# bldeng/AA-ADMM

Measured on AMD Instinct MI355X. Metric: ADMM iters/sec + time-to-eps (primal+dual residual), higher is better.
Workload: dtype f64

## Files before the change

aa-admm_amd/csrc/elastic.cpp:

```cpp
#include "elastic.hpp"

#include <algorithm>
#include <chrono>
#include <cmath>
#include <cstdio>
#include <cstdlib>
#include <cstring>
#include <memory>
#include <numeric>
#include <set>

#include "dense_gpu.hpp"
#include "spd_direct.hpp"

namespace aa {

ElasticSolver::~ElasticSolver() {
    if (fr_ev0_) { (void)hipEventDestroy(fr_ev0_); (void)hipEventDestroy(fr_ev1_); }
    if (fr_ev2_) (void)hipEventDestroy(fr_ev2_);
    drop_graph();
    if (ev_fork_) (void)hipEventDestroy(ev_fork_);
    if (ev_join_) (void)hipEventDestroy(ev_join_);
    if (side_) (void)hipStreamDestroy(side_);
    for (auto& kv : kstats_)
// ... 621 lines not shown
        auto pf = make_part_factor(P > 1 ? comm_ : nullptr, rank_, s());
        F = factor_on_device(A, tree, s(), pf.get());
    } catch (const Error&) {
        throw;
    } catch (const std::runtime_error& e) {
        throw Error(ERR_NUMERIC, e.what());
    }
    pipe_z_ = st_.variant == AA_VARIANT_Z && st_.acceleration_type == 1;
    if (const char* e = std::getenv("AA_Z_PIPELINE")) pipe_z_ = pipe_z_ && e[0] != '0';
    conc_ = pipe_z_ && !comm_;
    if (const char* e = std::getenv("AA_CONCURRENT")) conc_ = conc_ && e[0] != '0';
    win_u_ = conc_;
    if (const char* e = std::getenv("AA_Z_WINDOW")) win_u_ = win_u_ && e[0] != '0';
    comb_fused_ = true;
    if (const char* e = std::getenv("AA_COMB_FUSED")) comb_fused_ = e[0] != '0';
    stamp("factor");
    solver_.default_branches = (P == 1 && st_.variant == AA_VARIANT_Z) ? 2 : 1;
    solver_.build(F, s(), P > 1 ? &tree.part : nullptr, rank_, top_beg_, comm_, pipe_z_ ? 2 : 1,
                  st_.variant == AA_VARIANT_Z && st_.acceleration_type == 1);
    stamp("solver build + upload");

    std::vector<HostGroup> owned;
    nbg_ = 0;
    long long zmax = 0;
    if (P > 1) {
        std::vector<int> qpart(n, -1);
        for (int r = 0; r < P; ++r) for (int q = tree.part_beg[r]; q < tree.part_end[r]; ++q) qpart[q] = r;
        std::vector<long long> zr(P, 0);
        std::vector<int> br(P, 0);
        long long rr = 0;
// ... 98 lines not shown
            groups_[gi].d.spos = groups_[gi].spos.p;
        }
        Yslots_ = pos;
    }
    std::vector<double> xs(3 * (size_t)n), ms(n);
    for (int q = 0; q < n; ++q) {
        for (int j = 0; j < 3; ++j) xs[3 * (size_t)q + j] = x_[3 * (size_t)int2node_[q] + j];
        ms[q] = m3_[3 * (size_t)int2node_[q]];
    }
    xs_.upload(xs, s());
    vs_.alloc(3 * (size_t)n); vs_.zero(s());
    mass_.upload(ms, s());
    xfull_.alloc(3 * (size_t)n); xlast_.alloc(3 * (size_t)n); cxfull_.alloc(3 * (size_t)n);
    xfull_.zero(s()); xlast_.zero(s()); cxfull_.zero(s());
    xbar_.alloc(3 * (size_t)nf_); Mxbar_.alloc(3 * (size_t)nf_); b_.alloc(3 * (size_t)nf_);
    if (pipe_z_) b2_.alloc(3 * (size_t)nf_); dx_.alloc(3 * (size_t)nf_);
    z_.alloc(Z_); if (!win_u_) u_.alloc(Z_); y_.alloc(3 * std::max<long long>(1, Yslots_)); du_.alloc(Z_);
    if (st_.variant == AA_VARIANT_Z) { dz_.alloc(Z_); lastz_.alloc(Z_); cz_.alloc(Z_); }
    if (conc_) {
        du2_.alloc(Z_); dz2_.alloc(Z_); dx2_.alloc(3 * (size_t)nf_);
        ctrl_c_.alloc(1);
        lzq2_.alloc(2);
        AA_HIP(hipMemset(lzq2_.p, 0, 2 * sizeof(int)));
        if (!side_) AA_HIP(hipStreamCreateWithFlags(&side_, hipStreamNonBlocking));
        if (!ev_fork_) AA_HIP(hipEventCreateWithFlags(&ev_fork_, hipEventDisableTiming));
        if (!ev_join_) AA_HIP(hipEventCreateWithFlags(&ev_join_, hipEventDisableTiming));
    }
    nbg_ = std::max(1, nbg_);
    red_ab_.alloc(2 * (size_t)nbg_); red_ab_.zero(s());
    if (conc_) { red_c_.alloc(2 * (size_t)nbg_); red_c_.zero(s()); }
    pa_ = red_ab_.p; pb_ = red_ab_.p + nbg_;
    if (comm_) { red_gab_.alloc(2 * (size_t)nbg_); red_gab_.zero(s()); ga_ = red_gab_.p; gb_ = red_gab_.p + nbg_; }
    else { ga_ = pa_; gb_ = pb_; }
    ctrl_.alloc(1);
    lzq_.alloc(2);
    AA_HIP(hipMemset(lzq_.p, 0, 2 * sizeof(int)));
    if (const char* q = std::getenv("AA_LOCAL_QUEUE")) use_queue_ = q[0] != '0';
    lq_ = make_local_queue(ctx_->device, lzq_.p);
    if (conc_) {
        lq2_ = make_local_queue(ctx_->device, lzq2_.p);
    }
    if (const char* q = std::getenv("AA_LQ_STATS"); q && q[0] == '1') {
        lq_stats_.alloc(kLqStats);
        lq_stats_.zero(s());
        lq_.stats = lq_stats_.p;
    }
    if (conc_) lq2_.stats = lq_.stats;
    hist_cap_ = std::max(1, st_.admm_iters);
    hist_prim_.alloc(hist_cap_); hist_comb_.alloc(hist_cap_); hist_rej_.alloc(hist_cap_);
// ... 97 lines not shown
    zero(own_end_, top_beg_);
    if (rank_ != 0) zero(top_beg_, n_);
    comm_->allreduce_sum(v.p, v.p, 3 * (size_t)n_, s());
}

void ElasticSolver::upload_pins() {
    if (!pins_dirty_) return;
    std::vector<double> p(3 * (size_t)np_);
    int q = 0;
    for (auto& kv : pins_) { for (int j = 0; j < 3; ++j) p[3 * q + j] = kv.second[j]; ++q; }
    if (np_) {
        const size_t off = 3 * (size_t)nf_;
        AA_HIP(hipMemcpyAsync(xfull_.p + off, p.data(), p.size() * 8, hipMemcpyHostToDevice, s()));
        AA_HIP(hipMemcpyAsync(xlast_.p + off, p.data(), p.size() * 8, hipMemcpyHostToDevice, s()));
        AA_HIP(hipMemcpyAsync(cxfull_.p + off, p.data(), p.size() * 8, hipMemcpyHostToDevice, s()));
        AA_HIP(hipStreamSynchronize(s()));
    }
    pins_dirty_ = false;
}

void ElasticSolver::ev_begin(const char* name) {
    if (!instrument_) return;
    hipEvent_t e;
    AA_HIP(hipEventCreate(&e));
    AA_HIP(hipEventRecord(e, s()));
    kstats_[name].ev.push_back(e);
}
void ElasticSolver::ev_end(const char* name) { ev_begin(name); }

void ElasticSolver::local_z_all(const double* xfull, const double* u, double* z, double* y, int mode, bool red) {
// ... 100 lines not shown
        launch_aa_reduce(G, aa_cur_.p, Z_, aa_dF_.p, aa_dG_.p, c, aa_red_.p, aa_blocks_, cp, m, s(), ga_, gb_, nbg_,
                         hist_prim_.p, hist_comb_.p, hist_rej_.p);
        reduce_aa();
        launch_aa_solve(c, aag_, aa_blocks_, m, s());
        launch_aa_mix(G, aa_cur_.p, Z_, aa_dF_.p, aa_dG_.p, c, G, m, s(), comb_fused_);
        ev_end("aa");
    } else {
        launch_control(CTL_COMB_UX, c, ga_, gb_, nbg_, accel, hist_prim_.p, hist_comb_.p, hist_rej_.p, s());
    }
}

void ElasticSolver::enqueue_iteration_z(bool accel, int it) {
    const long long nx = 3LL * nf_;
    Ctrl* c = ctrl_.p;
    const bool pipe = accel && pipe_z_;
    double *duc = du_at(it), *dzc = dz_at(it), *dxc = dx_at(it);
    double *dup = du_at(it - 1), *dzp = dz_at(it - 1), *dxp = dx_at(it - 1);
    const bool side = pipe && it > 0 && conc_;
    auto side_pass = [&](hipStream_t st) {
        comb_finish_z(CTL_COMB_ZP, st, ctrl_c_.p, red_c_.p, red_c_.p + nbg_, &lq2_, dup, dzp);
    };
    double* u = u_at(it);
    const double* ui = win_u_ ? dup : u_.p;
    ev_begin("grad");
    for (auto& g : groups_) launch_u_and_y(g.d, xfull_.p, z_.p, u, u, y_.p, nf_, accel ? 1 : 0, 0, c, s(), g.var);
    ev_end("grad");
    ev_begin("rhs");
    launch_rhs(nf_, dt_ptr_.p, nullptr, nullptr, y_.p, Mxbar_.p, pdt2_, b_.p, c, 0, s());
    ev_end("rhs");
    if (pipe && it > 0) {
        ev_begin("solve");
        solver_.solve2(b_.p, xfull_.p, b2_.p, cxfull_.p, c, 0, s());
        ev_end("solve");
        if (side) {
            launch_ctrl_fork(c, ctrl_c_.p, s());
        } else {
            ev_begin("comb");
            comb_finish_z(CTL_COMB_ZP, s(), c, pa_, pb_, &lq_, dup, dzp);
            launch_copy(xfull_.p, dxp, nx, c, 2, s());
            ev_end("comb");
        }
    } else {
        ev_begin(pipe ? "solve1" : "solve");
        solver_.solve(b_.p, xfull_.p, c, 0, s());
        ev_end(pipe ? "solve1" : "solve");
    }
    auto prim_all = [&](const double* xf, const double* z, const double* zref, int redo) {
        int off = 0;
        for (auto& g : groups_) {
            launch_prim_z(g.d, xf, z, zref, nf_, redo, c, pa_, zref ? pb_ : nullptr, off, s());
            off += blocks_for(g.d.count);
        }
    };
    ev_begin("prim");
    prim_all(xfull_.p, z_.p, nullptr, 0);
    ev_end("prim");
    reduce_partials();
    launch_check_restore_z(c, ga_, nbg_, accel, win_u_ ? nullptr : u_.p, xfull_.p, z_.p, dup, dxp, dzp, Z_, nx, s());
    if (accel) {
        ev_begin("reject");
        for (auto& g : groups_) launch_u_and_y(g.d, xfull_.p, z_.p, ui, u, y_.p, nf_, 0, 1, c, s(), g.var);
        launch_rhs(nf_, dt_ptr_.p, nullptr, nullptr, y_.p, Mxbar_.p, pdt2_, b_.p, c, 1, s());
        solver_.solve(b_.p, xfull_.p, c, 1, s());
        prim_all(xfull_.p, z_.p, nullptr, 1);
        reduce_partials();
        ev_end("reject");
    }
    launch_control(CTL_PRIM_FINAL_Z, c, ga_, nullptr, nbg_, accel, hist_prim_.p, hist_comb_.p, hist_rej_.p, s());
    if (accel) {
        const int m = st_.anderson_m;
        auto copy_defaults = [&]() {
            ev_begin("copy");
            launch_copy(dxc, xfull_.p, nx, c, 0, s());
            if (!win_u_) launch_copy(duc, u_.p, Z_, c, 0, s());
            ev_end("copy");
        };
        if (instrument_) copy_defaults();
        ev_begin("local_z");
        local_z_all(xfull_.p, u, dzc, y_.p, LZ_NORMAL, false);
        ev_end("local_z");
        if (side && instrument_) {
            ev_begin("comb");
            side_pass(s());
// ... 40 lines not shown
    ev_end("local_z");
    prim_all(xfull_.p, z_.p, lastz_.p, 0);
    reduce_partials();
    launch_control(CTL_COMB_Z, c, ga_, gb_, nbg_, accel, hist_prim_.p, hist_comb_.p, hist_rej_.p, s());
}

void ElasticSolver::comb_finish_z(int op, hipStream_t st, Ctrl* c, double* pa, double* pb, const LocalQueue* q,
                                  const double* du, const double* dz) {
    const LocalQueue* lq = use_queue_ ? q : nullptr;
    auto fused = [&](const DevGroup& g) { return comb_fused_ && local_z_res_ok(g.d, lq); };
    for (auto& g : groups_) {
        if (fused(g)) launch_local_z_res(g.d, cxfull_.p, du, dz, cz_.p, nf_, c, st, lq, g.var);
        else launch_local_z(g.d, cxfull_.p, du, cz_.p, nullptr, nf_, st_.variant, LZ_NORMAL, c, nullptr, 0, st, lq, g.var,
                            mesh_table(g.d));
    }
    int off = 0;
    for (auto& g : groups_) {
        if (fused(g)) launch_prim_sum(g.d, cz_.p, c, pa, pb, off, st);
        else launch_prim_z(g.d, cxfull_.p, cz_.p, dz, nf_, 0, c, pa, pb, off, st);
        off += blocks_for(g.d.count);
    }
    if (st == s()) {
        reduce_partials();
        launch_control(op, c, ga_, gb_, nbg_, 1, hist_prim_.p, hist_comb_.p, hist_rej_.p, st);
    } else {
        launch_control(op, c, pa, pb, nbg_, 1, hist_prim_.p, hist_comb_.p, hist_rej_.p, st);
    }
}

void ElasticSolver::join_side() {
    if (join_wait_) AA_HIP(hipStreamWaitEvent(s(), ev_join_, 0));
    launch_ctrl_join(ctrl_.p, ctrl_c_.p, xfull_.p, join_dx_, 3LL * nf_, s());
}

void ElasticSolver::enqueue_comb_tail_z(int iters) {
    ev_begin("comb");
// ... 420 lines not shown
```

aa-admm_amd/csrc/elastic.hpp:

```cpp
#pragma once
#include <array>
#include <map>
#include <memory>
#include <string>
#include <vector>

#include "../../include/aa_admm.h"
#include "bending.hpp"
#include "comm.hpp"
#include "common.hpp"
#include "contact_friction.hpp"
#include "direct_solve.hpp"
#include "elastic_kernels.hpp"
#include "mesh_obstacle.hpp"
#include "mesh_refit.hpp"

namespace aa {

struct Context {
    int device = 0;
    hipStream_t stream = nullptr;
};

struct MeshObsBuffers {
// ... 200 lines not shown
    bool join_wait_ = false;
    double* join_dx_ = nullptr;
    void join_side();
    hipStream_t side_ = nullptr;
    hipEvent_t ev_fork_ = nullptr, ev_join_ = nullptr;
    DevBuf<Ctrl> ctrl_c_;
    DevBuf<int> lzq2_;
    LocalQueue lq2_;
    DevBuf<double> red_c_, du2_, dz2_, dx2_;
    double* du_at(int it) { return conc_ && (it & 1) ? du2_.p : du_.p; }
    double* dz_at(int it) { return conc_ && (it & 1) ? dz2_.p : dz_.p; }
    double* dx_at(int it) { return conc_ && (it & 1) ? dx2_.p : dx_.p; }
    bool win_u_ = false;
    double* u_at(int it) { return win_u_ ? du_at(it) : u_.p; }
    bool comb_fused_ = true;

    bool instrument_ = false;
    struct KStat { std::vector<hipEvent_t> ev; double bytes = 0; double total_ms = 0; int launches = 0; };
    std::map<std::string, KStat> kstats_;
    void ev_begin(const char* name);
    void ev_end(const char* name);

    void upload_pins();
    void prologue();
    void enqueue_iteration_ux(bool accel);
    void enqueue_iteration_z(bool accel, int it);
    void comb_finish_z(int op, hipStream_t st, Ctrl* c, double* pa, double* pb, const LocalQueue* q,
                       const double* du, const double* dz);
    void enqueue_comb_tail_z(int iters);
    void enqueue_iterations(int iters, bool accel);
// ... 8 lines not shown
```

aa-admm_amd/csrc/elastic_kernels.hip:

```cpp
#include <algorithm>
#include <cstdlib>

#include "common.hpp"
#include "device_lbfgs.hpp"
#include "device_prox.hpp"
#include "elastic_kernels.hpp"

namespace aa {

namespace {

__device__ __forceinline__ double wave_sum(double v) {
#pragma unroll
    for (int o = 32; o > 0; o >>= 1) v += __shfl_down(v, o, 64);
    return v;
}

__device__ __forceinline__ double block_sum(double v, double* sm) {
    v = wave_sum(v);
    const int lane = threadIdx.x & 63, wid = threadIdx.x >> 6;
    if (lane == 0) sm[wid] = v;
    __syncthreads();
    double r = 0;
    if (threadIdx.x == 0)
// ... 30 lines not shown
__device__ __forceinline__ bool record_iter(Ctrl* c, double* hp, double* hc, int* hr, double comb) {
    const int k = c->nrec;
    if (k < c->cap) {
        hp[k] = c->prim; hc[k] = comb; hr[k] = c->reject;
        if (c->hist_clock) c->hist_clock[k] = (long long)wall_clock64();
    }
    c->nrec = k + 1;
    if (k == 0) c->eps_abs = c->eps_rel * comb;
    return c->eps_rel > 0 && comb <= c->eps_abs;
}

__device__ __forceinline__ bool gated(const Ctrl* c, int gate_reject) {
    if (!c) return false;
    if (c->done) return true;
    return gate_reject && !c->reject;
}

template <int S>
__device__ __forceinline__ void gather_F(const GroupDev& g, int e, const double* __restrict__ xfull, int nf, double* F,
                                         double* Cp) {
    constexpr int NV = shape_nv(S), NC = shape_nc(S);
#pragma unroll
    for (int i = 0; i < 3 * NC; ++i) { F[i] = 0; Cp[i] = 0; }
#pragma unroll
    for (int a = 0; a < NV; ++a) {
        const int v = g.idx[(size_t)a * g.count + e];
        const double x0 = xfull[3 * (size_t)v], x1 = xfull[3 * (size_t)v + 1], x2 = xfull[3 * (size_t)v + 2];
        const bool pin = v >= nf;
#pragma unroll
        for (int c = 0; c < NC; ++c) {
// ... 92 lines not shown
}

template <class... V>
constexpr bool kVar = sizeof...(V) != 0;
__device__ __forceinline__ const GroupVar& var_of(const GroupVar& v) { return v; }
struct ResArgs {
    const double* zref;
};
template <class... V>
constexpr bool kRes = false;
template <class... V>
constexpr bool kRes<ResArgs, V...> = true;
__device__ __forceinline__ const GroupVar& var_of(const ResArgs&, const GroupVar& v) { return v; }
__device__ __forceinline__ const ResArgs& res_of(const ResArgs& r) { return r; }
__device__ __forceinline__ const ResArgs& res_of(const ResArgs& r, const GroupVar&) { return r; }
template <bool VAR>
struct LaneMat {};
template <>
struct LaneMat<true> {
    double mu = 0, lambda = 0, k = 0;
};

template <int S, int HYPER, class... V>
__global__ __launch_bounds__(kBlock) void k_local_z(GroupDev g, const double* __restrict__ xfull,
                                                    const double* __restrict__ u, double* __restrict__ z,
                                                    double* __restrict__ y, int nf, int variant, int mode, Ctrl* ctrl,
                                                    double* red, int red_off, V... gvp) {
    constexpr bool VAR = kVar<V...>;
    if (mode != LZ_INIT && gated(ctrl, mode == LZ_REDO)) return;
    __shared__ double sm[kBlock / 64];
// ... 493 lines not shown
            pa += r * r;
            pb += d * d;
            u[o] += r;
        }
    }
    const double sa = block_sum(pa, sm);
    const double sb = block_sum(pb, sm);
    if (threadIdx.x == 0) { red_a[red_off + blockIdx.x] = sa; red_b[red_off + blockIdx.x] = sb; }
}

template <int S, int HYPER, class... V>
__global__ __launch_bounds__(kBlock) void k_u_and_y(GroupDev g, const double* __restrict__ xfull,
                                                    const double* __restrict__ z, const double* uin, double* u,
                                                    double* __restrict__ y, int nf, int mode, int redo, Ctrl* ctrl,
                                                    V... gvp) {
    constexpr bool VAR = kVar<V...>;
    if (gated(ctrl, redo)) return;
    constexpr int NV = S == kShapeHinge ? 0 : shape_nv(S), D = 3 * shape_nc(S);
    const int e = blockIdx.x * blockDim.x + threadIdx.x;
    if (e >= g.count) return;
    double F[D], Cp[D], zz[D], uu[D];
    const double w = g.w[e];
    const double vol = (NV == 4 && mode == 1) ? g.vol[e] : 0.0;
    double mu = g.mu, lambda = g.lambda, k = g.k;
    if constexpr (VAR && NV == 4) {
        const GroupVar& gv = var_of(gvp...);
        if (mode == 1) { mu = gv.mu[e]; lambda = gv.lambda[e]; k = gv.k[e]; }
    }
#pragma unroll
    for (int i = 0; i < D; ++i) zz[i] = z[g.zoff + (size_t)i * g.count + e];
    if (mode != 1) {
#pragma unroll
        for (int i = 0; i < D; ++i) uu[i] = uin[g.zoff + (size_t)i * g.count + e];
    }
    if (mode == 1) {
        double gr[D];
        if constexpr (NV == 3 || NV == 1 || S == kShapeHinge) {
            if (ctrl) ctrl->fail = 2;
#pragma unroll
            for (int i = 0; i < D; ++i) gr[i] = 0;
        } else if constexpr (HYPER == 0) {
            dev::tet_linear_grad(zz, k * vol, gr);
        } else {
            dev::hyper_psi_grad(g.mat, mu, lambda, zz, gr);
#pragma unroll
            for (int i = 0; i < D; ++i) gr[i] *= vol;
        }
#pragma unroll
        for (int i = 0; i < D; ++i) uu[i] = gr[i] / w;
    }
    if (mode == 0) {
        gather_F<S>(g, e, xfull, nf, F, Cp);
#pragma unroll
        for (int i = 0; i < D; ++i) uu[i] += w * F[i] - w * zz[i];
    } else {
        gather_Cp<S>(g, e, xfull, nf, Cp);
    }
    if (mode != 2) {
#pragma unroll
        for (int i = 0; i < D; ++i) u[g.zoff + (size_t)i * g.count + e] = uu[i];
    }
    write_slots<S>(g, e, nf, w, zz, Cp, uu, y);
}

template <int S>
__global__ __launch_bounds__(kBlock) void k_prim_z(GroupDev g, const double* __restrict__ xfull,
                                                   const double* __restrict__ z, const double* __restrict__ zref,
                                                   int nf, int redo, Ctrl* ctrl, double* red_a, double* red_b,
                                                   int red_off) {
    if (gated(ctrl, redo)) return;
    __shared__ double sm[kBlock / 64];
    constexpr int D = 3 * shape_nc(S);
    const int e = blockIdx.x * blockDim.x + threadIdx.x;
    double pa = 0, pb = 0;
    if (e < g.count) {
        double F[D];
        gather_P<S>(g, e, xfull, F);
        const double w = g.w[e];
        double zi[D], zr[D];
#pragma unroll
        for (int i = 0; i < D; ++i) zi[i] = z[g.zoff + (size_t)i * g.count + e];
        if (zref) {
#pragma unroll
            for (int i = 0; i < D; ++i) zr[i] = zref[g.zoff + (size_t)i * g.count + e];
        }
#pragma unroll
        for (int i = 0; i < D; ++i) {
            const double r = w * (F[i] - zi[i]);
            pa += r * r;
            if (zref) { const double d = w * (zi[i] - zr[i]); pb += d * d; }
        }
    }
    const double sa = block_sum(pa, sm);
    const double sb = block_sum(pb, sm);
    if (threadIdx.x == 0) { red_a[red_off + blockIdx.x] = sa; if (red_b) red_b[red_off + blockIdx.x] = sb; }
}

__global__ __launch_bounds__(kBlock) void k_prim_sum(GroupDev g, const double* __restrict__ pe, Ctrl* ctrl,
                                                     double* red_a, double* red_b, int red_off) {
    if (gated(ctrl, 0)) return;
    __shared__ double sm[kBlock / 64];
    const int e = blockIdx.x * blockDim.x + threadIdx.x;
    double pa = 0, pb = 0;
    if (e < g.count) {
        pa = pe[g.zoff + e];
        pb = pe[g.zoff + (size_t)g.count + e];
    }
    const double sa = block_sum(pa, sm);
    const double sb = block_sum(pb, sm);
    if (threadIdx.x == 0) { red_a[red_off + blockIdx.x] = sa; red_b[red_off + blockIdx.x] = sb; }
}

template <int S>
__global__ __launch_bounds__(kBlock) void k_init_z(GroupDev g, const double* __restrict__ xfull, double* __restrict__ z) {
    constexpr int D = 3 * shape_nc(S);
    const int e = blockIdx.x * blockDim.x + threadIdx.x;
    if (e >= g.count) return;
    double F[D];
    gather_P<S>(g, e, xfull, F);
#pragma unroll
    for (int i = 0; i < D; ++i) z[g.zoff + (size_t)i * g.count + e] = F[i];
}

__global__ __launch_bounds__(kBlock) void k_rhs(int nf, const int* __restrict__ ptr, const int* __restrict__ row,
                                                const double* __restrict__ val, const double* __restrict__ y,
// ... 905 lines not shown
                        Ctrl* ctrl, hipStream_t s, const LocalQueue* queue, const GroupVar& var) {
    if (g.count == 0) return;
    const dim3 grid(std::min(blocks_for(g.count), std::max(1, queue->resident)));
    if (var)
        hipLaunchKernelGGL((k_local_z_hqf<4, false, ResArgs, GroupVar>), grid, dim3(kBlock), 0, s, g, xfull, u, pe, nullptr,
                           nf, (int)LZ_NORMAL, ctrl, queue->counter, queue->refill_lanes, queue->stats, ResArgs{zref}, var);
    else
        hipLaunchKernelGGL((k_local_z_hqf<4, false, ResArgs>), grid, dim3(kBlock), 0, s, g, xfull, u, pe, nullptr, nf,
                           (int)LZ_NORMAL, ctrl, queue->counter, queue->refill, queue->stats, ResArgs{zref});
    AA_CHECK_LAUNCH();
}

void launch_prim_sum(const GroupDev& g, const double* pe, Ctrl* ctrl, double* red_a, double* red_b, int red_off,
                     hipStream_t s) {
    if (g.count == 0) return;
    hipLaunchKernelGGL(k_prim_sum, dim3(blocks_for(g.count)), dim3(kBlock), 0, s, g, pe, ctrl, red_a, red_b, red_off);
    AA_CHECK_LAUNCH();
}

void launch_resid_update_u(const GroupDev& g, const double* xfull, const double* xlast, const double* z, double* u,
                           int nf, Ctrl* ctrl, double* red_a, double* red_b, int red_off, hipStream_t s) {
    if (g.count == 0) return;
    const int nb = blocks_for(g.count);
    if (g.kind == 3) hipLaunchKernelGGL(k_resid_u<kShapeHinge>, dim3(nb), dim3(kBlock), 0, s, g, xfull, xlast, z, u, nf, ctrl, red_a, red_b, red_off);
    else if (g.kind == 2) hipLaunchKernelGGL(k_resid_u<1>, dim3(nb), dim3(kBlock), 0, s, g, xfull, xlast, z, u, nf, ctrl, red_a, red_b, red_off);
    else if (g.kind == 1) hipLaunchKernelGGL(k_resid_u<3>, dim3(nb), dim3(kBlock), 0, s, g, xfull, xlast, z, u, nf, ctrl, red_a, red_b, red_off);
    else hipLaunchKernelGGL(k_resid_u<4>, dim3(nb), dim3(kBlock), 0, s, g, xfull, xlast, z, u, nf, ctrl, red_a, red_b, red_off);
    AA_CHECK_LAUNCH();
}

void launch_u_and_y(const GroupDev& g, const double* xfull, const double* z, const double* uin, double* u, double* y,
                    int nf, int mode, int redo, Ctrl* ctrl, hipStream_t s, const GroupVar& var) {
    if (g.count == 0) return;
    const int nb = blocks_for(g.count);
    if (g.kind == 3) hipLaunchKernelGGL((k_u_and_y<kShapeHinge, 0>), dim3(nb), dim3(kBlock), 0, s, g, xfull, z, uin, u, y, nf, mode, redo, ctrl);
    else if (g.kind == 2) hipLaunchKernelGGL((k_u_and_y<1, 0>), dim3(nb), dim3(kBlock), 0, s, g, xfull, z, uin, u, y, nf, mode, redo, ctrl);
    else if (g.kind == 1) hipLaunchKernelGGL((k_u_and_y<3, 0>), dim3(nb), dim3(kBlock), 0, s, g, xfull, z, uin, u, y, nf, mode, redo, ctrl);
    else if (g.mat == 0 && var) hipLaunchKernelGGL((k_u_and_y<4, 0, GroupVar>), dim3(nb), dim3(kBlock), 0, s, g, xfull, z, uin, u, y, nf, mode, redo, ctrl, var);
    else if (g.mat == 0) hipLaunchKernelGGL((k_u_and_y<4, 0>), dim3(nb), dim3(kBlock), 0, s, g, xfull, z, uin, u, y, nf, mode, redo, ctrl);
    else if (var) hipLaunchKernelGGL((k_u_and_y<4, 1, GroupVar>), dim3(nb), dim3(kBlock), 0, s, g, xfull, z, uin, u, y, nf, mode, redo, ctrl, var);
    else hipLaunchKernelGGL((k_u_and_y<4, 1>), dim3(nb), dim3(kBlock), 0, s, g, xfull, z, uin, u, y, nf, mode, redo, ctrl);
    AA_CHECK_LAUNCH();
}

void launch_prim_z(const GroupDev& g, const double* xfull, const double* z, const double* zref, int nf, int redo,
                   Ctrl* ctrl, double* red_a, double* red_b, int red_off, hipStream_t s) {
    if (g.count == 0) return;
    const int nb = blocks_for(g.count);
    if (g.kind == 3) hipLaunchKernelGGL(k_prim_z<kShapeHinge>, dim3(nb), dim3(kBlock), 0, s, g, xfull, z, zref, nf, redo, ctrl, red_a, red_b, red_off);
    else if (g.kind == 2) hipLaunchKernelGGL(k_prim_z<1>, dim3(nb), dim3(kBlock), 0, s, g, xfull, z, zref, nf, redo, ctrl, red_a, red_b, red_off);
    else if (g.kind == 1) hipLaunchKernelGGL(k_prim_z<3>, dim3(nb), dim3(kBlock), 0, s, g, xfull, z, zref, nf, redo, ctrl, red_a, red_b, red_off);
    else hipLaunchKernelGGL(k_prim_z<4>, dim3(nb), dim3(kBlock), 0, s, g, xfull, z, zref, nf, redo, ctrl, red_a, red_b, red_off);
    AA_CHECK_LAUNCH();
}

void launch_init_z(const GroupDev& g, const double* xfull, double* z, hipStream_t s) {
    if (g.count == 0) return;
    const int nb = blocks_for(g.count);
    if (g.kind == 3) hipLaunchKernelGGL(k_init_z<kShapeHinge>, dim3(nb), dim3(kBlock), 0, s, g, xfull, z);
    else if (g.kind == 2) hipLaunchKernelGGL(k_init_z<1>, dim3(nb), dim3(kBlock), 0, s, g, xfull, z);
    else if (g.kind == 1) hipLaunchKernelGGL(k_init_z<3>, dim3(nb), dim3(kBlock), 0, s, g, xfull, z);
    else hipLaunchKernelGGL(k_init_z<4>, dim3(nb), dim3(kBlock), 0, s, g, xfull, z);
    AA_CHECK_LAUNCH();
}

void launch_rhs(int nf, const int* ptr, const int* row, const double* val, const double* y, const double* Mxbar,
                double pdt2, double* b, Ctrl* ctrl, int gate_reject, hipStream_t s, const double* xsrc,
                double* xlast, const double* red_final, int nb_final) {
// ... 274 lines not shown
```

aa-admm_amd/csrc/elastic_kernels.hpp:

```cpp
#pragma once
#include <hip/hip_runtime.h>

#include "bvh.hpp"

namespace aa {

constexpr int kMaxM = 32;
constexpr double kCombEps = 1e-20;

struct GroupDev {
    int kind;
    int mat;
    int count;
    int nv, ncol, dim;
    int pinned;
    long long zoff;
    long long yrow;
    const int* idx;
    const int* spos;
    const double* G;
    const double* w;
    const double* vol;
    double mu, lambda, k, lmin, lmax;
    const double* obs;
// ... 60 lines not shown
    bool fused = false;
    bool split = false;
    unsigned long long* stats = nullptr;
};
constexpr int kLqStats = 104;
LocalQueue make_local_queue(int device, int* counter);
void launch_local_z(const GroupDev& g, const double* xfull, const double* u, double* z, double* y, int nf,
                    int variant, int mode, Ctrl* ctrl, double* red, int red_off, hipStream_t s,
                    const LocalQueue* queue = nullptr, const GroupVar& var = GroupVar(),
                    const MeshObsDev* meshes = nullptr);
bool local_z_res_ok(const GroupDev& g, const LocalQueue* queue);
void launch_local_z_res(const GroupDev& g, const double* xfull, const double* u, const double* zref, double* pe, int nf,
                        Ctrl* ctrl, hipStream_t s, const LocalQueue* queue, const GroupVar& var = GroupVar());
void launch_prim_sum(const GroupDev& g, const double* pe, Ctrl* ctrl, double* red_a, double* red_b, int red_off,
                     hipStream_t s);
void launch_resid_update_u(const GroupDev& g, const double* xfull, const double* xlast, const double* z, double* u,
                           int nf, Ctrl* ctrl, double* red_a, double* red_b, int red_off, hipStream_t s);
void launch_u_and_y(const GroupDev& g, const double* xfull, const double* z, const double* uin, double* u, double* y,
                    int nf, int mode, int redo, Ctrl* ctrl, hipStream_t s, const GroupVar& var = GroupVar());
void launch_prim_z(const GroupDev& g, const double* xfull, const double* z, const double* zref, int nf, int redo,
                   Ctrl* ctrl, double* red_a, double* red_b, int red_off, hipStream_t s);
void launch_rhs(int nf, const int* ptr, const int* row, const double* val, const double* y, const double* Mxbar,
                double pdt2, double* b, Ctrl* ctrl, int gate_reject, hipStream_t s,
                const double* xsrc = nullptr, double* xlast = nullptr, const double* red_final = nullptr,
                int nb_final = 0);
void launch_check_restore_z(Ctrl* ctrl, const double* red, int nb, int accel, double* u, double* x, double* z,
                            const double* du, const double* dx, const double* dz, long long nz, long long nx,
                            hipStream_t s);
void launch_check_restore_ux(Ctrl* ctrl, const double* red, int nb, int accel, double* u, double* x, double* cur,
                             const double* du, const double* dx, long long nz, long long nx, hipStream_t s);
void launch_restore_ux(double* u, double* x, double* cur, const double* du, const double* dx, long long nz,
                       long long nx, const Ctrl* ctrl, hipStream_t s);
enum CtlOp { CTL_PRIM_CHECK = 0, CTL_PRIM_FINAL = 1, CTL_COMB_UX = 2, CTL_PRIM_CHECK_Z = 3, CTL_PRIM_FINAL_Z = 4,
             CTL_COMB_Z = 5, CTL_COMB_ZP = 6 };
void launch_control(int op, Ctrl* ctrl, const double* red_a, const double* red_b, int nblocks, int accel,
                    double* hist_prim, double* hist_comb, int* hist_rej, hipStream_t s);
// ... 33 lines not shown
```

Measured before the change: 472.1.

## Fuse control reductions into last-block tails of primal-residual kernels

Adds a last-block-done ticket scheme so the final block of the last group's prim_z/prim_sum kernel reduces the per-block partials and updates the control struct. This removes the separate reduce_partials, check_restore and control kernel launches on the Z-accelerated path. The reject path is also restructured to read from the previous-iterate buffers and write z from within u_and_y, which replaces the separate restore step. The dx buffers are enlarged to include pinned nodes so they can stand in for xfull. The cost is atomics and fences in every block, plus the correctness risks of a grid-wide ticket protocol.

```diff
diff --git a/aa-admm_amd/csrc/elastic.cpp b/aa-admm_amd/csrc/elastic.cpp
--- a/aa-admm_amd/csrc/elastic.cpp
+++ b/aa-admm_amd/csrc/elastic.cpp
@@ -659,6 +659,8 @@
     if (const char* e = std::getenv("AA_Z_WINDOW")) win_u_ = win_u_ && e[0] != '0';
     comb_fused_ = true;
     if (const char* e = std::getenv("AA_COMB_FUSED")) comb_fused_ = e[0] != '0';
+    ctrl_fused_ = st_.variant == AA_VARIANT_Z && st_.acceleration_type == 1 && !comm_;
+    if (const char* e = std::getenv("AA_CTRL_FUSED")) ctrl_fused_ = ctrl_fused_ && e[0] != '0';
     stamp("factor");
     solver_.default_branches = (P == 1 && st_.variant == AA_VARIANT_Z) ? 2 : 1;
     solver_.build(F, s(), P > 1 ? &tree.part : nullptr, rank_, top_beg_, comm_, pipe_z_ ? 2 : 1,
@@ -787,11 +789,11 @@
     xfull_.alloc(3 * (size_t)n); xlast_.alloc(3 * (size_t)n); cxfull_.alloc(3 * (size_t)n);
     xfull_.zero(s()); xlast_.zero(s()); cxfull_.zero(s());
     xbar_.alloc(3 * (size_t)nf_); Mxbar_.alloc(3 * (size_t)nf_); b_.alloc(3 * (size_t)nf_);
-    if (pipe_z_) b2_.alloc(3 * (size_t)nf_); dx_.alloc(3 * (size_t)nf_);
+    if (pipe_z_) b2_.alloc(3 * (size_t)nf_); dx_.alloc(3 * (size_t)n); dx_.zero(s());
     z_.alloc(Z_); if (!win_u_) u_.alloc(Z_); y_.alloc(3 * std::max<long long>(1, Yslots_)); du_.alloc(Z_);
     if (st_.variant == AA_VARIANT_Z) { dz_.alloc(Z_); lastz_.alloc(Z_); cz_.alloc(Z_); }
     if (conc_) {
-        du2_.alloc(Z_); dz2_.alloc(Z_); dx2_.alloc(3 * (size_t)nf_);
+        du2_.alloc(Z_); dz2_.alloc(Z_); dx2_.alloc(3 * (size_t)n); dx2_.zero(s());
         ctrl_c_.alloc(1);
         lzq2_.alloc(2);
         AA_HIP(hipMemset(lzq2_.p, 0, 2 * sizeof(int)));
@@ -806,6 +808,13 @@
     if (comm_) { red_gab_.alloc(2 * (size_t)nbg_); red_gab_.zero(s()); ga_ = red_gab_.p; gb_ = red_gab_.p + nbg_; }
     else { ga_ = pa_; gb_ = pb_; }
     ctrl_.alloc(1);
+    last_group_ = -1;
+    for (int i = 0; i < (int)groups_.size(); ++i) if (groups_[i].d.count > 0) last_group_ = i;
+    if (last_group_ < 0) ctrl_fused_ = false;
+    if (ctrl_fused_) {
+        ticket_.alloc(2 * (size_t)kTicketInts);
+        AA_HIP(hipMemset(ticket_.p, 0, 2 * (size_t)kTicketInts * sizeof(int)));
+    }
     lzq_.alloc(2);
     AA_HIP(hipMemset(lzq_.p, 0, 2 * sizeof(int)));
     if (const char* q = std::getenv("AA_LOCAL_QUEUE")) use_queue_ = q[0] != '0';
@@ -933,6 +942,8 @@
         AA_HIP(hipMemcpyAsync(xfull_.p + off, p.data(), p.size() * 8, hipMemcpyHostToDevice, s()));
         AA_HIP(hipMemcpyAsync(xlast_.p + off, p.data(), p.size() * 8, hipMemcpyHostToDevice, s()));
         AA_HIP(hipMemcpyAsync(cxfull_.p + off, p.data(), p.size() * 8, hipMemcpyHostToDevice, s()));
+        AA_HIP(hipMemcpyAsync(dx_.p + off, p.data(), p.size() * 8, hipMemcpyHostToDevice, s()));
+        if (dx2_.p) AA_HIP(hipMemcpyAsync(dx2_.p + off, p.data(), p.size() * 8, hipMemcpyHostToDevice, s()));
         AA_HIP(hipStreamSynchronize(s()));
     }
     pins_dirty_ = false;
@@ -1063,6 +1074,7 @@
     const long long nx = 3LL * nf_;
     Ctrl* c = ctrl_.p;
     const bool pipe = accel && pipe_z_;
+    const bool cf = accel && ctrl_fused_;
     double *duc = du_at(it), *dzc = dz_at(it), *dxc = dx_at(it);
     double *dup = du_at(it - 1), *dzp = dz_at(it - 1), *dxp = dx_at(it - 1);
     const bool side = pipe && it > 0 && conc_;
@@ -1082,7 +1094,7 @@
         solver_.solve2(b_.p, xfull_.p, b2_.p, cxfull_.p, c, 0, s());
         ev_end("solve");
         if (side) {
-            launch_ctrl_fork(c, ctrl_c_.p, s());
+            if (!cf) launch_ctrl_fork(c, ctrl_c_.p, s());
         } else {
             ev_begin("comb");
             comb_finish_z(CTL_COMB_ZP, s(), c, pa_, pb_, &lq_, dup, dzp);
@@ -1094,28 +1106,44 @@
         solver_.solve(b_.p, xfull_.p, c, 0, s());
         ev_end(pipe ? "solve1" : "solve");
     }
-    auto prim_all = [&](const double* xf, const double* z, const double* zref, int redo) {
+    auto prim_all = [&](const double* xf, const double* z, const double* zref, int redo, const PrimTail* tail = nullptr) {
         int off = 0;
-        for (auto& g : groups_) {
-            launch_prim_z(g.d, xf, z, zref, nf_, redo, c, pa_, zref ? pb_ : nullptr, off, s());
+        for (int i = 0; i < (int)groups_.size(); ++i) {
+            auto& g = groups_[i];
+            if (tail && i == last_group_) launch_prim_z(g.d, xf, z, zref, nf_, redo, c, pa_, zref ? pb_ : nullptr, off, s(), *tail);
+            else launch_prim_z(g.d, xf, z, zref, nf_, redo, c, pa_, zref ? pb_ : nullptr, off, s());
             off += blocks_for(g.d.count);
         }
     };
-    ev_begin("prim");
-    prim_all(xfull_.p, z_.p, nullptr, 0);
-    ev_end("prim");
-    reduce_partials();
-    launch_check_restore_z(c, ga_, nbg_, accel, win_u_ ? nullptr : u_.p, xfull_.p, z_.p, dup, dxp, dzp, Z_, nx, s());
-    if (accel) {
+    if (cf) {
+        const PrimTail check{ticket_.p, pa_, nbg_, 1, side ? ctrl_c_.p : nullptr};
+        const PrimTail fin{ticket_.p, pa_, nbg_, 1, nullptr};
+        ev_begin("prim");
+        prim_all(xfull_.p, z_.p, nullptr, 0, &check);
+        ev_end("prim");
         ev_begin("reject");
-        for (auto& g : groups_) launch_u_and_y(g.d, xfull_.p, z_.p, ui, u, y_.p, nf_, 0, 1, c, s(), g.var);
+        for (auto& g : groups_) launch_u_and_y(g.d, dxp, dzp, dup, u, y_.p, nf_, 0, 1, c, s(), g.var, z_.p);
         launch_rhs(nf_, dt_ptr_.p, nullptr, nullptr, y_.p, Mxbar_.p, pdt2_, b_.p, c, 1, s());
         solver_.solve(b_.p, xfull_.p, c, 1, s());
-        prim_all(xfull_.p, z_.p, nullptr, 1);
+        prim_all(xfull_.p, z_.p, nullptr, 1, &fin);
+        ev_end("reject");
+    } else {
+        ev_begin("prim");
+        prim_all(xfull_.p, z_.p, nullptr, 0);
+        ev_end("prim");
         reduce_partials();
-        ev_end("reject");
-    }
-    launch_control(CTL_PRIM_FINAL_Z, c, ga_, nullptr, nbg_, accel, hist_prim_.p, hist_comb_.p, hist_rej_.p, s());
+        launch_check_restore_z(c, ga_, nbg_, accel, win_u_ ? nullptr : u_.p, xfull_.p, z_.p, dup, dxp, dzp, Z_, nx, s());
+        if (accel) {
+            ev_begin("reject");
+            for (auto& g : groups_) launch_u_and_y(g.d, xfull_.p, z_.p, ui, u, y_.p, nf_, 0, 1, c, s(), g.var);
+            launch_rhs(nf_, dt_ptr_.p, nullptr, nullptr, y_.p, Mxbar_.p, pdt2_, b_.p, c, 1, s());
+            solver_.solve(b_.p, xfull_.p, c, 1, s());
+            prim_all(xfull_.p, z_.p, nullptr, 1);
+            reduce_partials();
+            ev_end("reject");
+        }
+        launch_control(CTL_PRIM_FINAL_Z, c, ga_, nullptr, nbg_, accel, hist_prim_.p, hist_comb_.p, hist_rej_.p, s());
+    }
     if (accel) {
         const int m = st_.anderson_m;
         auto copy_defaults = [&]() {
@@ -1186,12 +1214,22 @@
         else launch_local_z(g.d, cxfull_.p, du, cz_.p, nullptr, nf_, st_.variant, LZ_NORMAL, c, nullptr, 0, st, lq, g.var,
                             mesh_table(g.d));
     }
+    const bool cf = ctrl_fused_;
+    const CombTail tail{cf ? ticket_.p + (st == s() ? 0 : kTicketInts) : nullptr, pa, pb, nbg_, op, hist_prim_.p, hist_comb_.p,
+                        hist_rej_.p};
     int off = 0;
-    for (auto& g : groups_) {
-        if (fused(g)) launch_prim_sum(g.d, cz_.p, c, pa, pb, off, st);
-        else launch_prim_z(g.d, cxfull_.p, cz_.p, dz, nf_, 0, c, pa, pb, off, st);
+    for (int i = 0; i < (int)groups_.size(); ++i) {
+        auto& g = groups_[i];
+        if (cf && i == last_group_) {
+            if (fused(g)) launch_prim_sum(g.d, cz_.p, c, pa, pb, off, st, tail);
+            else launch_prim_z(g.d, cxfull_.p, cz_.p, dz, nf_, 0, c, pa, pb, off, st, tail);
+        } else {
+            if (fused(g)) launch_prim_sum(g.d, cz_.p, c, pa, pb, off, st);
+            else launch_prim_z(g.d, cxfull_.p, cz_.p, dz, nf_, 0, c, pa, pb, off, st);
+        }
         off += blocks_for(g.d.count);
     }
+    if (cf) return;
     if (st == s()) {
         reduce_partials();
         launch_control(op, c, ga_, gb_, nbg_, 1, hist_prim_.p, hist_comb_.p, hist_rej_.p, st);
diff --git a/aa-admm_amd/csrc/elastic.hpp b/aa-admm_amd/csrc/elastic.hpp
--- a/aa-admm_amd/csrc/elastic.hpp
+++ b/aa-admm_amd/csrc/elastic.hpp
@@ -238,6 +238,9 @@
     bool win_u_ = false;
     double* u_at(int it) { return win_u_ ? du_at(it) : u_.p; }
     bool comb_fused_ = true;
+    bool ctrl_fused_ = false;
+    DevBuf<int> ticket_;
+    int last_group_ = -1;
 
     bool instrument_ = false;
     struct KStat { std::vector<hipEvent_t> ev; double bytes = 0; double total_ms = 0; int launches = 0; };
diff --git a/aa-admm_amd/csrc/elastic_kernels.hip b/aa-admm_amd/csrc/elastic_kernels.hip
--- a/aa-admm_amd/csrc/elastic_kernels.hip
+++ b/aa-admm_amd/csrc/elastic_kernels.hip
@@ -1,4 +1,5 @@
 #include <algorithm>
+#include <cstddef>
 #include <cstdlib>
 
 #include "common.hpp"
@@ -68,6 +69,117 @@
     if (!c) return false;
     if (c->done) return true;
     return gate_reject && !c->reject;
+}
+
+typedef __attribute__((address_space(1))) unsigned long long gu64;
+typedef __attribute__((address_space(1))) unsigned int gu32;
+__device__ __forceinline__ void st_through(double* p, double v) {
+    __hip_atomic_store((gu64*)p, (unsigned long long)__double_as_longlong(v), __ATOMIC_RELAXED, __HIP_MEMORY_SCOPE_AGENT);
+}
+__device__ __forceinline__ bool last_block(int* ticket, int* flag) {
+    if (threadIdx.x == 0) {
+        asm volatile("s_waitcnt vmcnt(0)" ::: "memory");
+        const unsigned nw = min(gridDim.x, (unsigned)kTicketWords), w = blockIdx.x % kTicketWords;
+        const unsigned mine = (gridDim.x - w + kTicketWords - 1) / kTicketWords;
+        gu32* wp = (gu32*)(ticket + (1 + w) * kTicketStride);
+        int last = 0;
+        if (__hip_atomic_fetch_add(wp, 1u, __ATOMIC_RELAXED, __HIP_MEMORY_SCOPE_AGENT) == mine - 1) {
+            __hip_atomic_store(wp, 0u, __ATOMIC_RELAXED, __HIP_MEMORY_SCOPE_AGENT);
+            last = __hip_atomic_fetch_add((gu32*)ticket, 1u, __ATOMIC_RELAXED, __HIP_MEMORY_SCOPE_AGENT) == nw - 1 ? 1 : 0;
+        }
+        if (last) {
+            __builtin_amdgcn_fence(__ATOMIC_ACQUIRE, "agent");
+            asm volatile("s_waitcnt vmcnt(0)" ::: "memory");
+            __hip_atomic_store((gu32*)ticket, 0u, __ATOMIC_RELAXED, __HIP_MEMORY_SCOPE_AGENT);
+        }
+        *flag = last;
+    }
+    __syncthreads();
+    return *flag != 0;
+}
+template <int NA>
+__device__ __forceinline__ void ctl_sum_1024(const double* const (&red)[NA], int nb, double* sm, double (&out)[NA]) {
+    const int lane = threadIdx.x & 63, wid = threadIdx.x >> 6;
+    constexpr int K = 4;
+    double a[NA][4];
+#pragma unroll
+    for (int s = 0; s < NA; ++s)
+#pragma unroll
+        for (int q = 0; q < 4; ++q) a[s][q] = 0;
+    for (int base = (int)threadIdx.x; base < nb; base += K * 1024) {
+        double v[NA][4][K];
+#pragma unroll
+        for (int s = 0; s < NA; ++s)
+#pragma unroll
+            for (int q = 0; q < 4; ++q)
+#pragma unroll
+                for (int k = 0; k < K; ++k) v[s][q][k] = red[s][min(base + k * 1024 + q * 256, nb - 1)];
+        __builtin_amdgcn_sched_barrier(0);
+#pragma unroll
+        for (int s = 0; s < NA; ++s)
+#pragma unroll
+            for (int q = 0; q < 4; ++q)
+#pragma unroll
+                for (int k = 0; k < K; ++k) a[s][q] = base + k * 1024 + q * 256 < nb ? a[s][q] + v[s][q][k] : a[s][q];
+    }
+#pragma unroll
+    for (int s = 0; s < NA; ++s)
+#pragma unroll
+        for (int q = 0; q < 4; ++q) {
+            const double w = wave_sum(a[s][q]);
+            if (lane == 0) sm[16 * s + 4 * q + wid] = w;
+        }
+    __syncthreads();
+#pragma unroll
+    for (int s = 0; s < NA; ++s) {
+        double r = 0;
+        if (threadIdx.x == 0)
+            for (int i = 0; i < 16; ++i) r += sm[16 * s + i];
+        out[s] = r;
+    }
+    __syncthreads();
+}
+
+__device__ __forceinline__ void ctl_head(const Ctrl* ctrl, const PrimTail& t) {
+    if (!t.side || blockIdx.x != 0) return;
+    const int* a = reinterpret_cast<const int*>(ctrl);
+    int* b = reinterpret_cast<int*>(t.side);
+    constexpr int pad = (int)(offsetof(Ctrl, pad_) / sizeof(int)), done = (int)(offsetof(Ctrl, done) / sizeof(int));
+    for (int i = threadIdx.x; i < (int)(sizeof(Ctrl) / sizeof(int)); i += blockDim.x) b[i] = a[i == pad ? done : i];
+}
+__device__ __forceinline__ void ctl_head(const Ctrl*, const CombTail&) {}
+
+__device__ __forceinline__ void ctl_tail(Ctrl* ctrl, int redo, const PrimTail& t) {
+    __shared__ double sm16[16];
+    __shared__ int flag;
+    if (!last_block(t.ticket, &flag)) return;
+    const double* const red[1] = {t.red};
+    double s[1];
+    ctl_sum_1024<1>(red, t.nb, sm16, s);
+    const double a = s[0];
+    if (threadIdx.x != 0) return;
+    const double prim = sqrt(a);
+    ctrl->prim = prim;
+    if (redo) { ctrl->prev_prim = prim; return; }
+    const int rej = (t.accel && ctrl->prev_prim < prim) ? 1 : 0;
+    ctrl->reject = rej;
+    if (rej) ctrl->nrej += 1;
+    else ctrl->prev_prim = prim;
+}
+
+__device__ __forceinline__ void ctl_tail(Ctrl* ctrl, int, const CombTail& t) {
+    __shared__ double sm32[32];
+    __shared__ int flag;
+    if (!last_block(t.ticket, &flag)) return;
+    const double* const red[2] = {t.red_a, t.red_b};
+    double s[2];
+    ctl_sum_1024<2>(red, t.nb, sm32, s);
+    if (threadIdx.x != 0) return;
+    const double comb = s[0] + s[1];
+    ctrl->iters_run += 1;
+    ctrl->comb = comb;
+    const bool eps = record_iter(ctrl, t.hist_prim, t.hist_comb, t.hist_rej, comb);
+    if (comb < kCombEps || eps) ctrl->done = t.op == CTL_COMB_ZP ? 2 : 1;
 }
 
 template <int S>
@@ -190,6 +302,16 @@
 __device__ __forceinline__ const GroupVar& var_of(const ResArgs&, const GroupVar& v) { return v; }
 __device__ __forceinline__ const ResArgs& res_of(const ResArgs& r) { return r; }
 __device__ __forceinline__ const ResArgs& res_of(const ResArgs& r, const GroupVar&) { return r; }
+struct ZOut {
+    double* z;
+};
+template <class... V>
+constexpr bool kZOut = false;
+template <class... V>
+constexpr bool kZOut<ZOut, V...> = true;
+__device__ __forceinline__ const GroupVar& var_of(const ZOut&, const GroupVar& v) { return v; }
+__device__ __forceinline__ const ZOut& zout_of(const ZOut& r) { return r; }
+__device__ __forceinline__ const ZOut& zout_of(const ZOut& r, const GroupVar&) { return r; }
 template <bool VAR>
 struct LaneMat {};
 template <>
@@ -713,7 +835,7 @@
                                                     const double* __restrict__ z, const double* uin, double* u,
                                                     double* __restrict__ y, int nf, int mode, int redo, Ctrl* ctrl,
                                                     V... gvp) {
-    constexpr bool VAR = kVar<V...>;
+    constexpr bool ZO = kZOut<V...>, VAR = sizeof...(V) > (ZO ? 1 : 0);
     if (gated(ctrl, redo)) return;
     constexpr int NV = S == kShapeHinge ? 0 : shape_nv(S), D = 3 * shape_nc(S);
     const int e = blockIdx.x * blockDim.x + threadIdx.x;
@@ -732,6 +854,11 @@
 #pragma unroll
         for (int i = 0; i < D; ++i) uu[i] = uin[g.zoff + (size_t)i * g.count + e];
     }
+    if constexpr (ZO) {
+        double* zo = zout_of(gvp...).z;
+#pragma unroll
+        for (int i = 0; i < D; ++i) zo[g.zoff + (size_t)i * g.count + e] = zz[i];
+    }
     if (mode == 1) {
         double gr[D];
         if constexpr (NV == 3 || NV == 1 || S == kShapeHinge) {
@@ -762,11 +889,12 @@
     write_slots<S>(g, e, nf, w, zz, Cp, uu, y);
 }
 
-template <int S>
+template <int S, class... T>
 __global__ __launch_bounds__(kBlock) void k_prim_z(GroupDev g, const double* __restrict__ xfull,
                                                    const double* __restrict__ z, const double* __restrict__ zref,
                                                    int nf, int redo, Ctrl* ctrl, double* red_a, double* red_b,
-                                                   int red_off) {
+                                                   int red_off, T... tail) {
+    if constexpr (sizeof...(T) != 0) ctl_head(ctrl, tail...);
     if (gated(ctrl, redo)) return;
     __shared__ double sm[kBlock / 64];
     constexpr int D = 3 * shape_nc(S);
@@ -792,11 +920,17 @@
     }
     const double sa = block_sum(pa, sm);
     const double sb = block_sum(pb, sm);
-    if (threadIdx.x == 0) { red_a[red_off + blockIdx.x] = sa; if (red_b) red_b[red_off + blockIdx.x] = sb; }
-}
-
+    if constexpr (sizeof...(T) == 0) {
+        if (threadIdx.x == 0) { red_a[red_off + blockIdx.x] = sa; if (red_b) red_b[red_off + blockIdx.x] = sb; }
+    } else {
+        if (threadIdx.x == 0) { st_through(red_a + red_off + blockIdx.x, sa); if (red_b) st_through(red_b + red_off + blockIdx.x, sb); }
+        ctl_tail(ctrl, redo, tail...);
+    }
+}
+
+template <class... T>
 __global__ __launch_bounds__(kBlock) void k_prim_sum(GroupDev g, const double* __restrict__ pe, Ctrl* ctrl,
-                                                     double* red_a, double* red_b, int red_off) {
+                                                     double* red_a, double* red_b, int red_off, T... tail) {
     if (gated(ctrl, 0)) return;
     __shared__ double sm[kBlock / 64];
     const int e = blockIdx.x * blockDim.x + threadIdx.x;
@@ -807,7 +941,12 @@
     }
     const double sa = block_sum(pa, sm);
     const double sb = block_sum(pb, sm);
-    if (threadIdx.x == 0) { red_a[red_off + blockIdx.x] = sa; red_b[red_off + blockIdx.x] = sb; }
+    if constexpr (sizeof...(T) == 0) {
+        if (threadIdx.x == 0) { red_a[red_off + blockIdx.x] = sa; red_b[red_off + blockIdx.x] = sb; }
+    } else {
+        if (threadIdx.x == 0) { st_through(red_a + red_off + blockIdx.x, sa); st_through(red_b + red_off + blockIdx.x, sb); }
+        ctl_tail(ctrl, 0, tail...);
+    }
 }
 
 template <int S>
@@ -1743,7 +1882,15 @@
 void launch_prim_sum(const GroupDev& g, const double* pe, Ctrl* ctrl, double* red_a, double* red_b, int red_off,
                      hipStream_t s) {
     if (g.count == 0) return;
-    hipLaunchKernelGGL(k_prim_sum, dim3(blocks_for(g.count)), dim3(kBlock), 0, s, g, pe, ctrl, red_a, red_b, red_off);
+    hipLaunchKernelGGL(k_prim_sum<>, dim3(blocks_for(g.count)), dim3(kBlock), 0, s, g, pe, ctrl, red_a, red_b, red_off);
+    AA_CHECK_LAUNCH();
+}
+
+void launch_prim_sum(const GroupDev& g, const double* pe, Ctrl* ctrl, double* red_a, double* red_b, int red_off,
+                     hipStream_t s, const CombTail& tail) {
+    if (g.count == 0) return;
+    hipLaunchKernelGGL(k_prim_sum<CombTail>, dim3(blocks_for(g.count)), dim3(kBlock), 0, s, g, pe, ctrl, red_a, red_b,
+                       red_off, tail);
     AA_CHECK_LAUNCH();
 }
 
@@ -1759,9 +1906,21 @@
 }
 
 void launch_u_and_y(const GroupDev& g, const double* xfull, const double* z, const double* uin, double* u, double* y,
-                    int nf, int mode, int redo, Ctrl* ctrl, hipStream_t s, const GroupVar& var) {
+                    int nf, int mode, int redo, Ctrl* ctrl, hipStream_t s, const GroupVar& var, double* zout) {
     if (g.count == 0) return;
     const int nb = blocks_for(g.count);
+    if (zout) {
+        const ZOut zo{zout};
+        if (g.kind == 3) hipLaunchKernelGGL((k_u_and_y<kShapeHinge, 0, ZOut>), dim3(nb), dim3(kBlock), 0, s, g, xfull, z, uin, u, y, nf, mode, redo, ctrl, zo);
+        else if (g.kind == 2) hipLaunchKernelGGL((k_u_and_y<1, 0, ZOut>), dim3(nb), dim3(kBlock), 0, s, g, xfull, z, uin, u, y, nf, mode, redo, ctrl, zo);
+        else if (g.kind == 1) hipLaunchKernelGGL((k_u_and_y<3, 0, ZOut>), dim3(nb), dim3(kBlock), 0, s, g, xfull, z, uin, u, y, nf, mode, redo, ctrl, zo);
+        else if (g.mat == 0 && var) hipLaunchKernelGGL((k_u_and_y<4, 0, ZOut, GroupVar>), dim3(nb), dim3(kBlock), 0, s, g, xfull, z, uin, u, y, nf, mode, redo, ctrl, zo, var);
+        else if (g.mat == 0) hipLaunchKernelGGL((k_u_and_y<4, 0, ZOut>), dim3(nb), dim3(kBlock), 0, s, g, xfull, z, uin, u, y, nf, mode, redo, ctrl, zo);
+        else if (var) hipLaunchKernelGGL((k_u_and_y<4, 1, ZOut, GroupVar>), dim3(nb), dim3(kBlock), 0, s, g, xfull, z, uin, u, y, nf, mode, redo, ctrl, zo, var);
+        else hipLaunchKernelGGL((k_u_and_y<4, 1, ZOut>), dim3(nb), dim3(kBlock), 0, s, g, xfull, z, uin, u, y, nf, mode, redo, ctrl, zo);
+        AA_CHECK_LAUNCH();
+        return;
+    }
     if (g.kind == 3) hipLaunchKernelGGL((k_u_and_y<kShapeHinge, 0>), dim3(nb), dim3(kBlock), 0, s, g, xfull, z, uin, u, y, nf, mode, redo, ctrl);
     else if (g.kind == 2) hipLaunchKernelGGL((k_u_and_y<1, 0>), dim3(nb), dim3(kBlock), 0, s, g, xfull, z, uin, u, y, nf, mode, redo, ctrl);
     else if (g.kind == 1) hipLaunchKernelGGL((k_u_and_y<3, 0>), dim3(nb), dim3(kBlock), 0, s, g, xfull, z, uin, u, y, nf, mode, redo, ctrl);
@@ -1781,6 +1940,27 @@
     else if (g.kind == 1) hipLaunchKernelGGL(k_prim_z<3>, dim3(nb), dim3(kBlock), 0, s, g, xfull, z, zref, nf, redo, ctrl, red_a, red_b, red_off);
     else hipLaunchKernelGGL(k_prim_z<4>, dim3(nb), dim3(kBlock), 0, s, g, xfull, z, zref, nf, redo, ctrl, red_a, red_b, red_off);
     AA_CHECK_LAUNCH();
+}
+
+template <class T>
+static void launch_prim_z_tail(const GroupDev& g, const double* xfull, const double* z, const double* zref, int nf,
+                               int redo, Ctrl* ctrl, double* red_a, double* red_b, int red_off, hipStream_t s,
+                               const T& tail) {
+    if (g.count == 0) return;
+    const int nb = blocks_for(g.count);
+    if (g.kind == 3) hipLaunchKernelGGL((k_prim_z<kShapeHinge, T>), dim3(nb), dim3(kBlock), 0, s, g, xfull, z, zref, nf, redo, ctrl, red_a, red_b, red_off, tail);
+    else if (g.kind == 2) hipLaunchKernelGGL((k_prim_z<1, T>), dim3(nb), dim3(kBlock), 0, s, g, xfull, z, zref, nf, redo, ctrl, red_a, red_b, red_off, tail);
+    else if (g.kind == 1) hipLaunchKernelGGL((k_prim_z<3, T>), dim3(nb), dim3(kBlock), 0, s, g, xfull, z, zref, nf, redo, ctrl, red_a, red_b, red_off, tail);
+    else hipLaunchKernelGGL((k_prim_z<4, T>), dim3(nb), dim3(kBlock), 0, s, g, xfull, z, zref, nf, redo, ctrl, red_a, red_b, red_off, tail);
+    AA_CHECK_LAUNCH();
+}
+void launch_prim_z(const GroupDev& g, const double* xfull, const double* z, const double* zref, int nf, int redo,
+                   Ctrl* ctrl, double* red_a, double* red_b, int red_off, hipStream_t s, const PrimTail& tail) {
+    launch_prim_z_tail(g, xfull, z, zref, nf, redo, ctrl, red_a, red_b, red_off, s, tail);
+}
+void launch_prim_z(const GroupDev& g, const double* xfull, const double* z, const double* zref, int nf, int redo,
+                   Ctrl* ctrl, double* red_a, double* red_b, int red_off, hipStream_t s, const CombTail& tail) {
+    launch_prim_z_tail(g, xfull, z, zref, nf, redo, ctrl, red_a, red_b, red_off, s, tail);
 }
 
 void launch_init_z(const GroupDev& g, const double* xfull, double* z, hipStream_t s) {
diff --git a/aa-admm_amd/csrc/elastic_kernels.hpp b/aa-admm_amd/csrc/elastic_kernels.hpp
--- a/aa-admm_amd/csrc/elastic_kernels.hpp
+++ b/aa-admm_amd/csrc/elastic_kernels.hpp
@@ -98,12 +98,37 @@
                         Ctrl* ctrl, hipStream_t s, const LocalQueue* queue, const GroupVar& var = GroupVar());
 void launch_prim_sum(const GroupDev& g, const double* pe, Ctrl* ctrl, double* red_a, double* red_b, int red_off,
                      hipStream_t s);
+constexpr int kTicketWords = 64, kTicketStride = 32, kTicketInts = (1 + kTicketWords) * kTicketStride;
+struct PrimTail {
+    int* ticket;
+    const double* red;
+    int nb;
+    int accel;
+    Ctrl* side;
+};
+struct CombTail {
+    int* ticket;
+    const double* red_a;
+    const double* red_b;
+    int nb;
+    int op;
+    double* hist_prim;
+    double* hist_comb;
+    int* hist_rej;
+};
+void launch_prim_sum(const GroupDev& g, const double* pe, Ctrl* ctrl, double* red_a, double* red_b, int red_off,
+                     hipStream_t s, const CombTail& tail);
 void launch_resid_update_u(const GroupDev& g, const double* xfull, const double* xlast, const double* z, double* u,
                            int nf, Ctrl* ctrl, double* red_a, double* red_b, int red_off, hipStream_t s);
 void launch_u_and_y(const GroupDev& g, const double* xfull, const double* z, const double* uin, double* u, double* y,
-                    int nf, int mode, int redo, Ctrl* ctrl, hipStream_t s, const GroupVar& var = GroupVar());
+                    int nf, int mode, int redo, Ctrl* ctrl, hipStream_t s, const GroupVar& var = GroupVar(),
+                    double* zout = nullptr);
 void launch_prim_z(const GroupDev& g, const double* xfull, const double* z, const double* zref, int nf, int redo,
                    Ctrl* ctrl, double* red_a, double* red_b, int red_off, hipStream_t s);
+void launch_prim_z(const GroupDev& g, const double* xfull, const double* z, const double* zref, int nf, int redo,
+                   Ctrl* ctrl, double* red_a, double* red_b, int red_off, hipStream_t s, const PrimTail& tail);
+void launch_prim_z(const GroupDev& g, const double* xfull, const double* z, const double* zref, int nf, int redo,
+                   Ctrl* ctrl, double* red_a, double* red_b, int red_off, hipStream_t s, const CombTail& tail);
 void launch_rhs(int nf, const int* ptr, const int* row, const double* val, const double* y, const double* Mxbar,
                 double pdt2, double* b, Ctrl* ctrl, int gate_reject, hipStream_t s,
                 const double* xsrc = nullptr, double* xlast = nullptr, const double* red_final = nullptr,
```

New measurement: 477.7, median of 4. No clear change (+1.2%).
